# yjh0410/YOLO-Nano

Measured on AMD Instinct MI355X. Metric: images/sec YOLO-Nano-1.0x 416x416 bs=32 inference (network + decode + NMS + host delivery), higher is better.
Workload: dtype f32 (split-f16 MFMA x3, fp32 accumulate); 1 GPU; YOLO-Nano-1.0x 416x416 bs=32/GPU fp32 inference, COCO 80-class head + NMS (BASELINE configs[1]); inputs resident in HBM, kept detections delivered to pinned host memory inside the timed region; global_batch=32, parallelism=image-sharded x1, no collective, rccl_ranks=1, launch_mode=eager, streams_per_gpu=4

## Files before the change

yolo-nano_amd/csrc/kernels_conv.hip:

```cpp
#include "yn_internal.h"
#include "yn_device.h"

#include <cstdio>
#include <mutex>
#include <set>
#include <string>

namespace ynk {

static thread_local const char* g_last_kernel = "";
const char* last_kernel_name() { return g_last_kernel; }
void set_last_kernel_name(const char* n) { g_last_kernel = n; }

bool g_log_lds = getenv("YN_LOG_LDS") != nullptr && atoi(getenv("YN_LOG_LDS")) != 0;
void note_launch_lds(const char* kernel, size_t dyn_lds, unsigned threads)
{
    static std::mutex mu;
    static std::set<std::string> seen;
    char line[512];
    snprintf(line, sizeof line, "yn_lds %s %zu %u", kernel, dyn_lds, threads);
    std::lock_guard<std::mutex> lk(mu);
    if (seen.insert(line).second) fprintf(stderr, "%s\n", line);
}

// ... 1013 lines not shown
        if (need <= maxnt) return need;
        for (int nt = maxnt; nt >= 1; --nt) if (nt32 % (nt * wn) == 0) return nt;
        return maxnt;
    };
    auto blocks = [&](int wm, int wn, int nt) {
        const long BM = 32 * wm, BN = 32 * nt * wn;
        return ((M + BM - 1) / BM) * ((Npad + BN - 1) / BN);
    };
    int wm = 4, wn = 1, nt = pick_nt(1, 4);
    if (blocks(wm, wn, nt) < 384) {
        const int nt2 = pick_nt(2, 2);
        if (blocks(2, 2, nt2) > blocks(wm, wn, nt)) { wm = 2; wn = 2; nt = nt2; }
        if (blocks(wm, wn, nt) < 256) {
            const int nt3 = pick_nt(4, 2);
            if (blocks(1, 4, nt3) > blocks(wm, wn, nt)) { wm = 1; wn = 4; nt = nt3; }
            if (blocks(wm, wn, nt) < 256 && nt > 1 && blocks(wm, wn, 1) > blocks(wm, wn, nt)) nt = 1;
        }
    }
    const bool one_shot = K <= 64;
    int idx = find_pw_cfg(wm, wn, nt, one_shot ? 32 : 16, one_shot ? 1 : 2);
    const TileCfg& c = g_pw_cfgs[idx];
    if (c.WM != wm || c.WN != wn || c.NT != nt) idx = find_pw_cfg(wm, wn, nt, 16, 2);
    return idx;
}

void launch_pw(const GemmArgs& a, hipStream_t s)
{
    int idx = a.cfg;
    if (idx == N_PW_CFGS + N_PWD_CFGS + N_PWS_CFGS) { if (launch_pw_pipe(a, s)) return; idx = -1; }
    if (a.Wsh && (idx < 0 || idx >= N_PW_CFGS + N_PWD_CFGS) && launch_pw_split(a, idx < 0 ? -1 : idx - N_PW_CFGS - N_PWD_CFGS, s)) return;
    if (idx >= N_PW_CFGS + N_PWD_CFGS) idx = -1;
    if (idx >= N_PW_CFGS && idx < N_PW_CFGS + N_PWD_CFGS && launch_pw_direct(a, idx - N_PW_CFGS, s)) return;
    if (idx < 0 || idx >= N_PW_CFGS) idx = choose_pw_cfg(a.M, a.K, a.Npad);
    const TileCfg& c = g_pw_cfgs[idx];
    const int BM = 32 * c.WM, BN = 32 * c.NT * c.WN;
    dim3 grid(xcd_grid((a.M + BM - 1) / BM) * ((a.Npad + BN - 1) / BN));
    g_last_kernel = g_pw_names[idx];
    int i = 0;
#define X(wm, wn, nt, kp, nb)                                                                              \
    if (i++ == idx) { hipLaunchKernelGGL((gemm_conv_kernel<wm, wn, nt, 0, kp, nb>), grid, dim3(256), 0, s, a); return; }
    YN_PW_CONFIGS(X)
#undef X
}

static void launch_gemm_3x3(const GemmArgs& a, hipStream_t s)
{
    const int nt32 = a.Npad / 32;
    if (nt32 % 3 == 0) {
        dim3 grid(xcd_grid((a.M + 127) / 128) * (a.Npad / 96));
        g_last_kernel = "gemm_conv_kernel<4,1,3,1,16,2>";
        hipLaunchKernelGGL((gemm_conv_kernel<4, 1, 3, 1, 16, 2>), grid, dim3(256), 0, s, a);
    } else {
        dim3 grid(xcd_grid((a.M + 127) / 128) * nt32);
        g_last_kernel = "gemm_conv_kernel<4,1,1,1,16,2>";
        hipLaunchKernelGGL((gemm_conv_kernel<4, 1, 1, 1, 16, 2>), grid, dim3(256), 0, s, a);
    }
}

void launch_conv3x3(const GemmArgs& a, hipStream_t s)
{
    const int nt32 = a.Npad / 32;
    const int NT = nt32 >= 3 && nt32 % 3 == 0 ? 3 : (nt32 % 2 == 0 ? 2 : 1);
    if (a.Wsh && a.Wsl && a.K == 96 && a.Npad == 96 && a.in_off == 0 && a.in_ld == 96 && (a.N & 3) == 0 && (a.out_ld & 3) == 0 && (a.out_off & 3) == 0 &&
        conv3x3_split_lds(a.W, 1, 1) <= 160 * 1024) {
        static unsigned long long attr_s = 0;
        if (attr_pending(attr_s)) {
            (void)hipFuncSetAttribute(reinterpret_cast<const void*>(conv3x3_split_kernel<3, 2>), hipFuncAttributeMaxDynamicSharedMemorySize, 160 * 1024);
            (void)hipFuncSetAttribute(reinterpret_cast<const void*>(conv3x3_split_kernel<1, 2, 1>), hipFuncAttributeMaxDynamicSharedMemorySize, 160 * 1024);
            (void)hipFuncSetAttribute(reinterpret_cast<const void*>(conv3x3_split_kernel<1, 1, 9>), hipFuncAttributeMaxDynamicSharedMemorySize, 160 * 1024);
            (void)hipFuncSetAttribute(reinterpret_cast<const void*>(conv3x3_split_kernel<1, 1, 3>), hipFuncAttributeMaxDynamicSharedMemorySize, 160 * 1024);
            (void)hipFuncSetAttribute(reinterpret_cast<const void*>(conv3x3_split_kernel<1, 1, 1>), hipFuncAttributeMaxDynamicSharedMemorySize, 160 * 1024);
        }
        const int tiles = (a.M + 127) / 128;
        if (tiles >= 256) {
            g_last_kernel = "conv3x3_split_kernel<3,2>";
            hipLaunchKernelGGL((conv3x3_split_kernel<3, 2>), dim3(xcd_grid(tiles), 1), dim3(256), conv3x3_split_lds(a.W, 3, 2), s, a);
        } else if (tiles * 3 >= 256) {
            if (tiles * 2 >= 256) {
                g_last_kernel = "conv3x3_split_kernel<3,2>";
                hipLaunchKernelGGL((conv3x3_split_kernel<3, 2>), dim3(xcd_grid(tiles), 1), dim3(256), conv3x3_split_lds(a.W, 3, 2), s, a);
                return;
            }
            g_last_kernel = "conv3x3_split_kernel<1,2>";
            hipLaunchKernelGGL((conv3x3_split_kernel<1, 2, 1>), dim3(xcd_grid(tiles), 3), dim3(256), conv3x3_split_lds(a.W, 1, 2, 1), s, a);
        } else if (conv3x3_split_lds(a.W, 1, 1, 9) <= 160 * 1024) {
            g_last_kernel = "conv3x3_split_kernel<1,1,9>";
            hipLaunchKernelGGL((conv3x3_split_kernel<1, 1, 9>), dim3(xcd_grid(tiles), 3), dim3(256), conv3x3_split_lds(a.W, 1, 1, 9), s, a);
        } else if (conv3x3_split_lds(a.W, 1, 1, 3) <= 160 * 1024) {
            g_last_kernel = "conv3x3_split_kernel<1,1,3>";
            hipLaunchKernelGGL((conv3x3_split_kernel<1, 1, 3>), dim3(xcd_grid(tiles), 3), dim3(256), conv3x3_split_lds(a.W, 1, 1, 3), s, a);
        } else {
            g_last_kernel = "conv3x3_split_kernel<1,1,1>";
            hipLaunchKernelGGL((conv3x3_split_kernel<1, 1, 1>), dim3(xcd_grid(tiles), 3), dim3(256), conv3x3_split_lds(a.W, 1, 1, 1), s, a);
        }
        return;
    }
    if (a.K == 96 && NT == 3 && a.in_off == 0 && a.in_ld == 96 && (a.N & 3) == 0 && (a.out_ld & 3) == 0 && (a.out_off & 3) == 0 &&
        conv3x3_halo_tap_lds(a.W, 96, 3) <= 160 * 1024) {
        static unsigned long long attr_t = 0;
        if (attr_pending(attr_t)) {
            (void)hipFuncSetAttribute(reinterpret_cast<const void*>(conv3x3_halo_tap_kernel<3, 96, 1>), hipFuncAttributeMaxDynamicSharedMemorySize, 160 * 1024);
            (void)hipFuncSetAttribute(reinterpret_cast<const void*>(conv3x3_halo_tap_kernel<1, 96, 1>), hipFuncAttributeMaxDynamicSharedMemorySize, 160 * 1024);
            (void)hipFuncSetAttribute(reinterpret_cast<const void*>(conv3x3_halo_tap_kernel<1, 96, 2>), hipFuncAttributeMaxDynamicSharedMemorySize, 160 * 1024);
        }
        const int tiles = (a.M + 127) / 128;
        if (tiles * (a.Npad / 96) >= 256) {
            g_last_kernel = "conv3x3_halo_tap_kernel<3,96,1>";
            hipLaunchKernelGGL((conv3x3_halo_tap_kernel<3, 96, 1>), dim3(xcd_grid(tiles), a.Npad / 96), dim3(256), conv3x3_halo_tap_lds(a.W, 96, 3), s, a);
        } else if (conv3x3_halo_tap_lds(a.W, 96, 1) > 80 * 1024 && conv3x3_halo_tap_lds(a.W, 96, 1, 2) <= 80 * 1024) {
            g_last_kernel = "conv3x3_halo_tap_kernel<1,96,2>";
            hipLaunchKernelGGL((conv3x3_halo_tap_kernel<1, 96, 2>), dim3(xcd_grid(tiles), a.Npad / 32), dim3(256), conv3x3_halo_tap_lds(a.W, 96, 1, 2), s, a);
        } else {
            g_last_kernel = "conv3x3_halo_tap_kernel<1,96,1>";
            hipLaunchKernelGGL((conv3x3_halo_tap_kernel<1, 96, 1>), dim3(xcd_grid(tiles), a.Npad / 32), dim3(256), conv3x3_halo_tap_lds(a.W, 96, 1), s, a);
        }
        return;
    }
    const size_t lds = (a.K % 32 == 0 && a.in_off == 0) ? conv3x3_halo_lds(a.W, a.K, NT) : (size_t)1 << 30;
    if (lds <= 160 * 1024 && a.K / 2 <= 256) {
        static unsigned long long attr = 0;
        if (attr_pending(attr)) {
            (void)hipFuncSetAttribute(reinterpret_cast<const void*>(conv3x3_halo_kernel<1>), hipFuncAttributeMaxDynamicSharedMemorySize, 160 * 1024);
            (void)hipFuncSetAttribute(reinterpret_cast<const void*>(conv3x3_halo_kernel<2>), hipFuncAttributeMaxDynamicSharedMemorySize, 160 * 1024);
            (void)hipFuncSetAttribute(reinterpret_cast<const void*>(conv3x3_halo_kernel<3>), hipFuncAttributeMaxDynamicSharedMemorySize, 160 * 1024);
        }
        dim3 grid((a.M + 127) / 128, a.Npad / (32 * NT));
        if (NT == 3) { g_last_kernel = "conv3x3_halo_kernel<3>"; hipLaunchKernelGGL(conv3x3_halo_kernel<3>, grid, dim3(256), lds, s, a); }
        else if (NT == 2) { g_last_kernel = "conv3x3_halo_kernel<2>"; hipLaunchKernelGGL(conv3x3_halo_kernel<2>, grid, dim3(256), lds, s, a); }
        else { g_last_kernel = "conv3x3_halo_kernel<1>"; hipLaunchKernelGGL(conv3x3_halo_kernel<1>, grid, dim3(256), lds, s, a); }
        return;
    }
    launch_gemm_3x3(a, s);
}

template <int STRIDE, int VEC, int R>
__device__ __forceinline__ void dwconv3x3_block(const DwArgs& a, unsigned bid, unsigned nblocks)
{
    typedef typename VecT<VEC>::type vec;
    constexpr int NCOL = STRIDE == 1 ? R + 2 : 2 * R + 1;
    const int Ho = (a.H - 1) / STRIDE + 1, Wo = (a.W - 1) / STRIDE + 1;
    const int cv_n = a.C / VEC, segs = (Wo + R - 1) / R;
    const int total = a.B * Ho * segs * cv_n;
    const int i = xcd_block(bid, nblocks) * 256 + threadIdx.x;
    if (i >= total) return;
    const int cv = i % cv_n;
    int q = i / cv_n;
    const int seg = q % segs; q /= segs;
    const int oy = q % Ho, b = q / Ho;
    const int c = cv * VEC, ox0 = seg * R;
    vec col[3][NCOL];
#pragma unroll
    for (int ky = 0; ky < 3; ++ky) {
        const int iy = oy * STRIDE - 1 + ky;
        const bool yok = iy >= 0 && iy < a.H;
        const float* row = a.in + ((size_t)(b * a.H + (yok ? iy : 0)) * a.W) * a.in_ld + a.in_off + c;
#pragma unroll
        for (int j = 0; j < NCOL; ++j) {
            const int ix = ox0 * STRIDE - 1 + j;
            const unsigned mk = opaque_mask(yok && ix >= 0 && ix < a.W);
            col[ky][j] = vmask(*reinterpret_cast<const vec*>(row + (size_t)(ix < 0 ? 0 : (ix >= a.W ? a.W - 1 : ix)) * a.in_ld), mk);
        }
    }
    vec w[9];
#pragma unroll
    for (int k = 0; k < 9; ++k) w[k] = *reinterpret_cast<const vec*>(a.w + k * a.C + c);
    const vec bias = *reinterpret_cast<const vec*>(a.bias + c);
    float* orow = a.out + ((size_t)(b * Ho + oy) * Wo) * a.out_ld + a.out_off + c;
#pragma unroll
    for (int o = 0; o < R; ++o) {
        if (ox0 + o >= Wo) break;
        vec acc = bias;
#pragma unroll
        for (int ky = 0; ky < 3; ++ky)
#pragma unroll
            for (int kx = 0; kx < 3; ++kx) vfma(acc, col[ky][o * STRIDE + kx], w[ky * 3 + kx]);
        *reinterpret_cast<vec*>(orow + (size_t)(ox0 + o) * a.out_ld) = vact(acc, a.act);
    }
}

template <int STRIDE, int VEC, int R>
__global__ __launch_bounds__(256) void dwconv3x3_kernel(DwArgs a) { dwconv3x3_block<STRIDE, VEC, R>(a, blockIdx.x, gridDim.x); }

template <int R>
__global__ __launch_bounds__(256) void dwconv3x3_group_kernel(Group<DwArgs> g)
{
    unsigned local, nb;
    const int p = group_problem(g.first, blockIdx.x, local, nb);
    dwconv3x3_block<1, 4, R>(g.a[p], local, nb);
}

bool dw_group_ok(const DwArgs* a, int n)
{
    if (n < 1 || n > YN_GROUP_MAX) return false;
    for (int p = 0; p < n; ++p)
        if (a[p].stride != 1 || (a[p].C % 4) || (a[p].in_ld % 4) || (a[p].in_off % 4) || (a[p].out_ld % 4) || (a[p].out_off % 4)) return false;
    return true;
}

void launch_dw_group(const DwArgs* a, int n, hipStream_t s)
{
    auto blocks_for = [&](const DwArgs& q, int r) { return (unsigned)(((long)q.B * q.H * ((q.W + r - 1) / r) * (q.C / 4) + 255) / 256); };
    unsigned all4 = 0;
    for (int p = 0; p < n; ++p) all4 += blocks_for(a[p], 4);
    const int R = all4 >= 1024 ? 4 : 2;
    Group<DwArgs> g{};
    unsigned tot = 0;
    for (int p = 0; p < YN_GROUP_MAX; ++p) {
        g.first[p] = tot;
        if (p < n) { g.a[p] = a[p]; tot += xcd_grid(blocks_for(a[p], R)); }
    }
    g.first[YN_GROUP_MAX] = tot;
    if (R == 4) { g_last_kernel = "dwconv3x3_group_kernel<4>"; hipLaunchKernelGGL(dwconv3x3_group_kernel<4>, dim3(tot), dim3(256), 0, s, g); }
    else        { g_last_kernel = "dwconv3x3_group_kernel<2>"; hipLaunchKernelGGL(dwconv3x3_group_kernel<2>, dim3(tot), dim3(256), 0, s, g); }
}

void launch_dw(const DwArgs& a, hipStream_t s)
{
    const int Ho = (a.H - 1) / a.stride + 1, Wo = (a.W - 1) / a.stride + 1;
    const bool v4 = (a.C % 4 == 0) && (a.in_ld % 4 == 0) && (a.in_off % 4 == 0) && (a.out_ld % 4 == 0) && (a.out_off % 4 == 0);
    auto blocks_for = [&](int vec, int r) { return ((long)a.B * Ho * ((Wo + r - 1) / r) * (a.C / vec) + 255) / 256; };
#define YN_DW(ST, V, R) { g_last_kernel = "dwconv3x3_kernel<" #ST "," #V "," #R ">"; \
        hipLaunchKernelGGL((dwconv3x3_kernel<ST, V, R>), dim3(xcd_grid((unsigned)blocks_for(V, R))), dim3(256), 0, s, a); return; }
    if (a.stride == 1) {
        if (v4) { if (blocks_for(4, 4) >= 1024) YN_DW(1, 4, 4) else YN_DW(1, 4, 2) }
        else    { if (blocks_for(2, 8) >= 1024) YN_DW(1, 2, 8) else YN_DW(1, 2, 4) }
    } else {
        if (v4) { if (blocks_for(4, 4) >= 1024) YN_DW(2, 4, 4) else YN_DW(2, 4, 2) }
        else    { if (blocks_for(2, 4) >= 1024) YN_DW(2, 2, 4) else YN_DW(2, 2, 2) }
    }
#undef YN_DW
}

template <int COUT>
__global__ __launch_bounds__(256) void stem_kernel(const float* __restrict__ x, int B, int H, int W,
                                                    const float* __restrict__ w, const float* __restrict__ bias,
                                                    int act, float* __restrict__ y)
{
    __shared__ __attribute__((aligned(16))) float ws[28 * COUT];
    for (int i = threadIdx.x; i < 27 * COUT; i += 256) ws[i] = w[i];
    for (int i = threadIdx.x; i < COUT; i += 256) ws[27 * COUT + i] = bias[i];
    __syncthreads();
    const int Ho = (H - 1) / 2 + 1, Wo = (W - 1) / 2 + 1, Wp = (Wo + 1) / 2;
    const long total = (long)B * Ho * Wp;
    const long p = (long)blockIdx.x * 256 + threadIdx.x;
    if (p >= total) return;
    const int opx = (int)(p % Wp);
    const long q = p / Wp;
    const int oy = (int)(q % Ho);
    const int b = (int)(q / Ho);
    const int ox0 = opx * 2;
    const bool has1 = ox0 + 1 < Wo;
    float acc0[COUT], acc1[COUT];
#pragma unroll
    for (int co = 0; co < COUT; ++co) { acc0[co] = ws[27 * COUT + co]; acc1[co] = acc0[co]; }
#pragma unroll 1
    for (int cy = 0; cy < 9; ++cy) {
        const int ci = cy / 3, ky = cy - ci * 3;
        const float* xp = x + ((size_t)b * 3 + ci) * H * W;
        {
            const int iy = oy * 2 - 1 + ky;
            const bool rowok = iy >= 0 && iy < H;
            float in[5];
#pragma unroll
            for (int j = 0; j < 5; ++j) {
                const int ix = ox0 * 2 - 1 + j;
                in[j] = (rowok && ix >= 0 && ix < W) ? xp[(size_t)iy * W + ix] : 0.0f;
            }
#pragma unroll
            for (int kx = 0; kx < 3; ++kx) {
                const float4* wr = reinterpret_cast<const float4*>(ws + ((ci * 3 + ky) * 3 + kx) * COUT);
#pragma unroll
                for (int c4 = 0; c4 < COUT / 4; ++c4) {
                    const float4 wv = wr[c4];
                    acc0[c4 * 4 + 0] += in[kx] * wv.x; acc0[c4 * 4 + 1] += in[kx] * wv.y;
                    acc0[c4 * 4 + 2] += in[kx] * wv.z; acc0[c4 * 4 + 3] += in[kx] * wv.w;
                    acc1[c4 * 4 + 0] += in[kx + 2] * wv.x; acc1[c4 * 4 + 1] += in[kx + 2] * wv.y;
                    acc1[c4 * 4 + 2] += in[kx + 2] * wv.z; acc1[c4 * 4 + 3] += in[kx + 2] * wv.w;
                }
            }
        }
    }
    float* yo = y + (((size_t)b * Ho + oy) * Wo + ox0) * COUT;
#pragma unroll
    for (int co = 0; co < COUT; co += 4)
        *reinterpret_cast<float4*>(yo + co) = make_float4(apply_act(acc0[co], act), apply_act(acc0[co + 1], act),
                                                          apply_act(acc0[co + 2], act), apply_act(acc0[co + 3], act));
    if (has1) {
#pragma unroll
        for (int co = 0; co < COUT; co += 4)
            *reinterpret_cast<float4*>(yo + COUT + co) = make_float4(apply_act(acc1[co], act), apply_act(acc1[co + 1], act),
                                                                     apply_act(acc1[co + 2], act), apply_act(acc1[co + 3], act));
    }
}

void launch_stem(const float* x, int B, int H, int W, const float* w, const float* bias, int Cout, int act, float* y, hipStream_t s)
{
    const int Ho = (H - 1) / 2 + 1, Wo = (W - 1) / 2 + 1;
    const long total = (long)B * Ho * ((Wo + 1) / 2);
    const unsigned blocks = (unsigned)((total + 255) / 256);
    g_last_kernel = "stem_kernel<24>";
    if (Cout == 24) hipLaunchKernelGGL(stem_kernel<24>, dim3(blocks), dim3(256), 0, s, x, B, H, W, w, bias, act, y);
}

template <int COUT>
__global__ __launch_bounds__(256) void stem_pool_kernel(const float* __restrict__ x, int B, int H, int W,
                                                         const float* __restrict__ w, const float* __restrict__ bias,
                                                         int act, float* __restrict__ y)
{
    constexpr int PR = 8, PC = 7, CR = 2 * PR + 1, CC = 2 * PC + 1;
    __shared__ __attribute__((aligned(16))) float ct[CR * CC * COUT];
    const int Hc = (H - 1) / 2 + 1, Wc = (W - 1) / 2 + 1;
    const int Hp = (Hc - 1) / 2 + 1, Wp = (Wc - 1) / 2 + 1;
    const int tiles_x = (Wp + PC - 1) / PC, tiles_y = (Hp + PR - 1) / PR;
    const int vb = (int)xcd_block(blockIdx.x, gridDim.x);
    if (vb >= tiles_x * tiles_y * B) return;
    const int tile = vb % (tiles_x * tiles_y), b = vb / (tiles_x * tiles_y);
    const int py0 = (tile / tiles_x) * PR, px0 = (tile % tiles_x) * PC;
    const int t = threadIdx.x;
    const int r = t / CC, c = t - r * CC;
    const int cy = 2 * py0 - 1 + r, cx = 2 * px0 - 1 + c;
    const bool live = t < CR * CC && cy >= 0 && cy < Hc && cx >= 0 && cx < Wc;
    float in[27];
    {
        const int cyc = live ? cy : 0, cxc = live ? cx : 0;
#pragma unroll
        for (int q = 0; q < 9; ++q) {
            const int ci = q / 3, ky = q - ci * 3;
            const float* xp = x + ((size_t)b * 3 + ci) * H * W;
            const int iy = cyc * 2 - 1 + ky;
            const bool rowok = live && iy >= 0 && iy < H;
            const float* xr = xp + (size_t)(iy < 0 ? 0 : (iy >= H ? H - 1 : iy)) * W;
#pragma unroll
            for (int k = 0; k < 3; ++k) {
                const int ix = cxc * 2 - 1 + k;
                const unsigned mk = opaque_mask(rowok && ix >= 0 && ix < W);
                in[q * 3 + k] = __uint_as_float(__float_as_uint(xr[ix < 0 ? 0 : (ix >= W ? W - 1 : ix)]) & mk);
            }
        }
    }
    float acc[COUT];
#pragma unroll
    for (int co = 0; co < COUT; ++co) acc[co] = bias[co];
#pragma unroll
    for (int i = 0; i < 27; ++i) {
#pragma unroll
        for (int co = 0; co < COUT; ++co) acc[co] += in[i] * w[i * COUT + co];
    }
#pragma unroll
    for (int co = 0; co < COUT; ++co) acc[co] = live ? apply_act(acc[co], act) : -INFINITY;
    if (t < CR * CC) {
#pragma unroll
        for (int co = 0; co < COUT; co += 4)
            *reinterpret_cast<float4*>(ct + t * COUT + co) = make_float4(acc[co], acc[co + 1], acc[co + 2], acc[co + 3]);
    }
    __syncthreads();
    constexpr int C4 = COUT / 4;
    for (int i = t; i < PR * PC * C4; i += 256) {
        const int c4 = i % C4, pp = i / C4;
        const int pr = pp / PC, pc = pp - pr * PC;
        const int py = py0 + pr, px = px0 + pc;
        if (py >= Hp || px >= Wp) continue;
        float4 m = make_float4(-INFINITY, -INFINITY, -INFINITY, -INFINITY);
#pragma unroll
        for (int dy = 0; dy < 3; ++dy)
#pragma unroll
            for (int dx = 0; dx < 3; ++dx) {
                const float4 v = *reinterpret_cast<const float4*>(ct + ((2 * pr + dy) * CC + 2 * pc + dx) * COUT + c4 * 4);
                m.x = fmaxf(m.x, v.x); m.y = fmaxf(m.y, v.y); m.z = fmaxf(m.z, v.z); m.w = fmaxf(m.w, v.w);
            }
        *reinterpret_cast<float4*>(y + (((size_t)b * Hp + py) * Wp + px) * COUT + c4 * 4) = m;
    }
}

void launch_stem_pool(const float* x, int B, int H, int W, const float* w, const float* bias, int Cout, int act, float* y, hipStream_t s)
{
    const int Hc = (H - 1) / 2 + 1, Wc = (W - 1) / 2 + 1, Hp = (Hc - 1) / 2 + 1, Wp = (Wc - 1) / 2 + 1;
    const int tiles = ((Wp + 6) / 7) * ((Hp + 7) / 8);
    g_last_kernel = "stem_pool_kernel<24>";
    if (Cout == 24) hipLaunchKernelGGL(stem_pool_kernel<24>, dim3(xcd_grid((unsigned)(tiles * B))), dim3(256), 0, s, x, B, H, W, w, bias, act, y);
}

__global__ __launch_bounds__(256) void maxpool_kernel(const float* __restrict__ x, int B, int H, int W, int C, float* __restrict__ y)
{
    const int Ho = (H - 1) / 2 + 1, Wo = (W - 1) / 2 + 1;
    const int c4n = C >> 2;
    const long total = (long)B * Ho * Wo * c4n;
    for (long i = (long)blockIdx.x * 256 + threadIdx.x; i < total; i += (long)gridDim.x * 256) {
        const int c4 = (int)(i % c4n);
        const long p = i / c4n;
        const int ox = (int)(p % Wo);
        const long q = p / Wo;
        const int oy = (int)(q % Ho);
        const int b = (int)(q / Ho);
        float4 m = make_float4(-INFINITY, -INFINITY, -INFINITY, -INFINITY);
#pragma unroll
        for (int ky = 0; ky < 3; ++ky) {
            const int iy = oy * 2 - 1 + ky;
            if (iy < 0 || iy >= H) continue;
#pragma unroll
            for (int kx = 0; kx < 3; ++kx) {
                const int ix = ox * 2 - 1 + kx;
                if (ix < 0 || ix >= W) continue;
                const float4 v = *reinterpret_cast<const float4*>(x + ((size_t)(b * H + iy) * W + ix) * C + c4 * 4);
                m.x = fmaxf(m.x, v.x); m.y = fmaxf(m.y, v.y); m.z = fmaxf(m.z, v.z); m.w = fmaxf(m.w, v.w);
            }
        }
        *reinterpret_cast<float4*>(y + (size_t)p * C + c4 * 4) = m;
    }
}

void launch_maxpool(const float* x, int B, int H, int W, int C, float* y, hipStream_t s)
{
    const int Ho = (H - 1) / 2 + 1, Wo = (W - 1) / 2 + 1;
    const long total = (long)B * Ho * Wo * (C >> 2);
    long blocks = (total + 255) / 256;
    if (blocks > 256 * 32) blocks = 256 * 32;
    if (blocks < 1) blocks = 1;
    g_last_kernel = "maxpool_kernel";
    hipLaunchKernelGGL(maxpool_kernel, dim3((unsigned)blocks), dim3(256), 0, s, x, B, H, W, C, y);
}

__global__ void nchw_to_nhwc_kernel(const float* __restrict__ x, int B, int C, int HW, float* __restrict__ y)
{
    __shared__ float tile[32][33];
    const int b = blockIdx.z;
    const int p0 = blockIdx.x * 32, c0 = blockIdx.y * 32;
    const int tx = threadIdx.x & 31, ty = threadIdx.x >> 5;
    for (int r = ty; r < 32; r += 8) {
        const int c = c0 + r, p = p0 + tx;
        tile[r][tx] = (c < C && p < HW) ? x[((size_t)b * C + c) * HW + p] : 0.0f;
    }
    __syncthreads();
    for (int r = ty; r < 32; r += 8) {
        const int p = p0 + r, c = c0 + tx;
        if (p < HW && c < C) y[((size_t)b * HW + p) * C + c] = tile[tx][r];
    }
}

void launch_nchw_to_nhwc(const float* x, int B, int C, int H, int W, float* y, hipStream_t s)
{
    const int HW = H * W;
    dim3 grid((HW + 31) / 32, (C + 31) / 32, B);
    hipLaunchKernelGGL(nchw_to_nhwc_kernel, grid, dim3(256), 0, s, x, B, C, HW, y);
}

void launch_nhwc_to_nchw(const float* x, int B, int C, int H, int W, float* y, hipStream_t s)
{
    const int HW = H * W;
    dim3 grid((C + 31) / 32, (HW + 31) / 32, B);
    hipLaunchKernelGGL(nchw_to_nhwc_kernel, grid, dim3(256), 0, s, x, B, HW, C, y);
}

__global__ void fold_pack_kernel(FoldArgs a)
{
    const int per_out = (a.kind == 1) ? a.kk : a.Cin * a.kk;
    const int total = a.Cout * per_out;
    const int i = blockIdx.x * 256 + threadIdx.x;
    if (i < a.Cout) {
        const int co = i;
        float f = 1.0f, bv = a.b ? a.b[co] : 0.0f;
        if (a.gamma) {
            f = a.gamma[co] / sqrtf(a.var[co] + a.eps);
            bv = (bv - a.mean[co]) * f + a.beta[co];
        }
        if (a.b_ref) a.b_ref[co] = bv;
        a.b_packed[co] = bv;
    }
    if (i >= total) return;
    const int co = i / per_out, r = i - co * per_out;
    float f = 1.0f;
    if (a.gamma) f = a.gamma[co] / sqrtf(a.var[co] + a.eps);
    const float v = a.w[i] * f;
    if (a.w_ref) a.w_ref[i] = v;
    if (a.kind == 1) {
        a.w_packed[r * a.Cout + co] = v;
    } else if (a.kind == 2) {
        a.w_packed[r * a.Cout + co] = v;
    } else {
        const int ci = r / a.kk, tap = r - ci * a.kk;
        const int k = tap * a.Cin + ci;
        a.w_packed[((size_t)(k >> 1) * a.Npad + co) * 2 + (k & 1)] = v;
        if (a.ws_hi) {
            if (a.w_ovf && !(fabsf(v) < 65504.0f)) atomicOr(a.w_ovf, 1u);
            const _Float16 hi = (_Float16)v, lo = split_lo(v, hi);
            const size_t o = (((size_t)tap * ((a.Cin + 7) >> 3) + (ci >> 3)) * a.Npad + co) * 8 + (ci & 7);
            reinterpret_cast<_Float16*>(a.ws_hi)[o] = hi;
            reinterpret_cast<_Float16*>(a.ws_lo)[o] = lo;
        }
    }
}

void launch_fold_pack(const FoldArgs& a, hipStream_t s)
{
    const int per_out = (a.kind == 1) ? a.kk : a.Cin * a.kk;
    int total = a.Cout * per_out;
    if (total < a.Cout) total = a.Cout;
    hipLaunchKernelGGL(fold_pack_kernel, dim3((total + 255) / 256), dim3(256), 0, s, a);
}

}
```

Baseline: 52770 images/s.

## Use paired float2 input loads with DPP neighbor exchange in stem+pool kernel

Measured after the change: 53420 images/s (median of 6 runs). 1.2% higher.

```diff
diff --git a/yolo-nano_amd/csrc/kernels_conv.hip b/yolo-nano_amd/csrc/kernels_conv.hip
--- a/yolo-nano_amd/csrc/kernels_conv.hip
+++ b/yolo-nano_amd/csrc/kernels_conv.hip
@@ -1339,13 +1339,21 @@
     if (Cout == 24) hipLaunchKernelGGL(stem_kernel<24>, dim3(blocks), dim3(256), 0, s, x, B, H, W, w, bias, act, y);
 }
 
+constexpr int STEM_POOL_C0_SPLIT = 15;
+constexpr int STEM_POOL_PIN = 9;
+__device__ __forceinline__ float mul_then_add(float a, float b, float c)
+{
+#pragma clang fp contract(off)
+    return c + a * b;
+}
+
 template <int COUT>
-__global__ __launch_bounds__(256) void stem_pool_kernel(const float* __restrict__ x, int B, int H, int W,
+__global__ __launch_bounds__(256) __attribute__((amdgpu_waves_per_eu(6, 6))) void stem_pool_kernel(const float* __restrict__ x, int B, int H, int W,
                                                          const float* __restrict__ w, const float* __restrict__ bias,
                                                          int act, float* __restrict__ y)
 {
     constexpr int PR = 8, PC = 7, CR = 2 * PR + 1, CC = 2 * PC + 1;
-    __shared__ __attribute__((aligned(16))) float ct[CR * CC * COUT];
+    __shared__ __attribute__((aligned(16))) float ct[256 * COUT];
     const int Hc = (H - 1) / 2 + 1, Wc = (W - 1) / 2 + 1;
     const int Hp = (Hc - 1) / 2 + 1, Wp = (Wc - 1) / 2 + 1;
     const int tiles_x = (Wp + PC - 1) / PC, tiles_y = (Hp + PR - 1) / PR;
@@ -1358,8 +1366,49 @@
     const int cy = 2 * py0 - 1 + r, cx = 2 * px0 - 1 + c;
     const bool live = t < CR * CC && cy >= 0 && cy < Hc && cx >= 0 && cx < Wc;
     float in[27];
-    {
-        const int cyc = live ? cy : 0, cxc = live ? cx : 0;
+    const int cyc = live ? cy : 0, cxc = live ? cx : 0;
+    if ((W & 1) == 0 && (reinterpret_cast<uintptr_t>(x) & 7) == 0 && (size_t)H * W <= (1u << 28)) {
+        asm volatile("; YN_STEM_PAIRED_BEGIN");
+        const bool edge = c == 0 || (t & 63) == 0;
+        const char* xb = reinterpret_cast<const char*>(x + (size_t)b * 3 * H * W);
+        const unsigned plane = (unsigned)H * (unsigned)W * 4u;
+        unsigned off[3];
+#pragma unroll
+        for (int ky = 0; ky < 3; ++ky) {
+            const int iy = cyc * 2 - 1 + ky;
+            off[ky] = ((unsigned)(iy < 0 ? 0 : (iy >= H ? H - 1 : iy)) * (unsigned)W + (unsigned)cxc * 2u) * 4u;
+        }
+#pragma unroll
+        for (int q = 0; q < 9; ++q) {
+            const int ci = q / 3, ky = q - ci * 3;
+            const float2 p = *reinterpret_cast<const float2*>(xb + ci * plane + off[ky]);
+            in[q * 3 + 1] = p.x;
+            in[q * 3 + 2] = p.y;
+            in[q * 3] = __int_as_float(__builtin_amdgcn_update_dpp(0, __float_as_int(p.y), 0x138, 0xf, 0xf, true));
+        }
+        if (edge) {
+            const unsigned back = cxc > 0 ? 4u : 0u;
+#pragma unroll
+            for (int q = 0; q < 9; ++q) {
+                const int ci = q / 3, ky = q - ci * 3;
+                in[q * 3] = *reinterpret_cast<const float*>(xb + ci * plane + (off[ky] - back));
+            }
+        }
+#pragma unroll
+        for (int ky = 0; ky < 3; ++ky) {
+            const int iy = cyc * 2 - 1 + ky;
+            const bool rowok = live && iy >= 0 && iy < H;
+            const unsigned mk = opaque_mask(rowok), ml = opaque_mask(rowok && cxc > 0);
+#pragma unroll
+            for (int ci = 0; ci < 3; ++ci) {
+                const int q = ci * 3 + ky;
+                in[q * 3] = __uint_as_float(__float_as_uint(in[q * 3]) & ml);
+                in[q * 3 + 1] = __uint_as_float(__float_as_uint(in[q * 3 + 1]) & mk);
+                in[q * 3 + 2] = __uint_as_float(__float_as_uint(in[q * 3 + 2]) & mk);
+            }
+        }
+        asm volatile("; YN_STEM_PAIRED_END");
+    } else {
 #pragma unroll
         for (int q = 0; q < 9; ++q) {
             const int ci = q / 3, ky = q - ci * 3;
@@ -1375,23 +1424,54 @@
             }
         }
     }
-    float acc[COUT];
-#pragma unroll
-    for (int co = 0; co < COUT; ++co) acc[co] = bias[co];
+    typedef float f4 __attribute__((ext_vector_type(4)));
+    constexpr int C4 = COUT / 4;
+    f4 acc[C4];
+#pragma unroll
+    for (int g = 0; g < C4; ++g) {
+        f4 bv = f4{bias[g * 4], bias[g * 4 + 1], bias[g * 4 + 2], bias[g * 4 + 3]};
+        asm volatile("" : "+s"(bv));
+#pragma unroll
+        for (int k = 0; k < 4; ++k) acc[g][k] = live ? bv[k] : -INFINITY;
+    }
 #pragma unroll
     for (int i = 0; i < 27; ++i) {
-#pragma unroll
-        for (int co = 0; co < COUT; ++co) acc[co] += in[i] * w[i * COUT + co];
-    }
-#pragma unroll
-    for (int co = 0; co < COUT; ++co) acc[co] = live ? apply_act(acc[co], act) : -INFINITY;
-    if (t < CR * CC) {
-#pragma unroll
-        for (int co = 0; co < COUT; co += 4)
-            *reinterpret_cast<float4*>(ct + t * COUT + co) = make_float4(acc[co], acc[co + 1], acc[co + 2], acc[co + 3]);
-    }
-    __syncthreads();
-    constexpr int C4 = COUT / 4;
+        const float a0 = acc[0].x;
+#pragma unroll
+        for (int g = 0; g < C4; ++g) {
+            const float* wi = w + i * COUT + g * 4;
+            acc[g] = __builtin_elementwise_fma(f4{in[i], in[i], in[i], in[i]}, f4{wi[0], wi[1], wi[2], wi[3]}, acc[g]);
+        }
+        if (i >= STEM_POOL_C0_SPLIT) acc[0].x = mul_then_add(in[i], w[i * COUT], a0);
+        if (i % STEM_POOL_PIN == STEM_POOL_PIN - 1 && i != 26) asm volatile("" : "+v"(acc[0]), "+v"(acc[1]), "+v"(acc[2]), "+v"(acc[3]), "+v"(acc[4]), "+v"(acc[5]));
+    }
+    auto put_tile = [&]() {
+#pragma unroll
+        for (int g = 0; g < C4; ++g) *reinterpret_cast<f4*>(ct + t * COUT + g * 4) = acc[g];
+        __syncthreads();
+    };
+    if (act == 1) {
+        const float floor = live ? 0.0f : -INFINITY;
+#pragma unroll
+        for (int g = 0; g < C4; ++g)
+#pragma unroll
+            for (int k = 0; k < 4; ++k) {
+                float v = acc[g][k];
+                asm("v_max_f32 %0, %1, %2" : "=v"(v) : "v"(v), "v"(floor));
+                acc[g][k] = v;
+            }
+        put_tile();
+    } else if (act == 2) {
+#pragma unroll
+        for (int g = 0; g < C4; ++g) {
+            const f4 neg = acc[g] * 0.1f;
+#pragma unroll
+            for (int k = 0; k < 4; ++k) acc[g][k] = acc[g][k] > 0.0f ? acc[g][k] : neg[k];
+        }
+        put_tile();
+    } else {
+        put_tile();
+    }
     for (int i = t; i < PR * PC * C4; i += 256) {
         const int c4 = i % C4, pp = i / C4;
         const int pr = pp / PC, pc = pp - pr * PC;
```
